# advait/c4a0

Hardware: AMD Instinct MI355X
Metric: self-play games/sec (and MCTS sims/sec) at n_mcts=100 (higher is better)
Workload: dtype bf16

## Files before the change

c4a0_amd/csrc/c4_head_gemm.hip:

```cpp
#include <hip/hip_runtime.h>
#include <stdint.h>

#include <string>
#include <type_traits>

#include "../../include/c4a0_hip.h"
#include "c4_grouped.hpp"
#include "c4_host.hpp"
#include "c4_timeline.hpp"

namespace {

typedef __bf16 bf16x8 __attribute__((ext_vector_type(8)));
typedef __bf16 bf16x4 __attribute__((ext_vector_type(4)));
typedef float f32x4 __attribute__((ext_vector_type(4)));

constexpr int BK = 64;

struct GemmParams {
  const uint16_t* x;
  const uint16_t* w;
  const float* bias;
  uint16_t* y;
  uint32_t M, N, K, ldx, ldy, relu;
  uint32_t xcd_mask, xcd_shift, xn_log2, rm, rn, rn_magic;
};

#define C4_GEMM_ARGS const uint16_t* __restrict__ a_x, const uint16_t* __restrict__ a_w, const float* __restrict__ a_bias, uint16_t* __restrict__ a_y, \
                     uint32_t a_m, uint32_t a_nk, uint32_t a_ld, uint32_t a_flags, uint32_t a_rmrn, uint32_t a_magic
#define C4_GEMM_UNPACK()                                                                                                              \
  GemmParams p;                                                                                                                        \
  p.x = a_x; p.w = a_w; p.bias = a_bias; p.y = a_y; p.M = a_m; p.N = a_nk & 0xFFFFu; p.K = a_nk >> 16; p.ldx = a_ld & 0xFFFFu;         \
  p.ldy = a_ld >> 16; p.relu = a_flags & 0xFFu; p.xn_log2 = (a_flags >> 8) & 0xFFu; p.xcd_mask = (a_flags >> 16) & 0xFFu;              \
  p.xcd_shift = a_flags >> 24; p.rm = a_rmrn & 0xFFFFu; p.rn = a_rmrn >> 16; p.rn_magic = a_magic

__host__ __device__ __forceinline__ void tile_of_block(uint32_t blk, uint32_t xcd_mask, uint32_t xcd_shift, uint32_t xn_log2, uint32_t rm, uint32_t rn,
                                                       uint32_t rn_magic, int& tm, int& tn) {
  const uint32_t xcd = blk & xcd_mask, idx = blk >> xcd_shift;
  const uint32_t qn = rn == 1u ? idx : (uint32_t)(((uint64_t)idx * rn_magic) >> 32);
  tm = (int)((xcd >> xn_log2) * rm + qn);
  tn = (int)((xcd & ((1u << xn_log2) - 1u)) * rn + (idx - qn * rn));
}

template <int N>
__device__ __forceinline__ void wait_vmcnt() { asm volatile("s_waitcnt vmcnt(%0)" ::"n"(N) : "memory"); }

#if defined(C4_PHASE_STAMPS) && !defined(C4_GEMM_CLOCK)
#define C4_GEMM_CLOCK
#endif
#ifdef C4_GEMM_CLOCK
__device__ unsigned long long c4_gemm_clk[16];
#define C4_CLK_DECL() unsigned long long clk_ts[8]; unsigned long long clk_c0 = 0, clk_c1 = 0
#define C4_GSTAMP(i) do { clk_ts[i] = __builtin_amdgcn_s_memrealtime(); } while (0)
#define C4_CLK_BEGIN() do { clk_c0 = __builtin_amdgcn_s_memtime(); } while (0)
#define C4_CLK_END() do { clk_c1 = __builtin_amdgcn_s_memtime(); } while (0)
#ifdef C4_PHASE_STAMPS
#define C4_CLK_SAMPLE() true
#else
#define C4_CLK_SAMPLE() ((blockIdx.x & 31) == 5)
#endif
#define C4_CLK_FLUSH()                                                                                       \
  do {                                                                                                       \
    if (threadIdx.x == 0 && C4_CLK_SAMPLE()) {                                                               \
      atomicAdd(&c4_gemm_clk[0], clk_c1 - clk_c0);                                                           \
      atomicAdd(&c4_gemm_clk[1], clk_ts[3] - clk_ts[1]);                                                     \
      atomicAdd(&c4_gemm_clk[2], 1ull);                                                                      \
      if (C4_CLK_PHASES) {                                                                                   \
        for (int i_ = 0; i_ < 7; i_++) atomicAdd(&c4_gemm_clk[4 + i_], clk_ts[i_ + 1] - clk_ts[i_]);         \
        atomicMin(&c4_gemm_clk[12], clk_ts[0]);                                                              \
        atomicMax(&c4_gemm_clk[13], clk_ts[7]);                                                              \
      }                                                                                                      \
    }                                                                                                        \
  } while (0)
#ifdef C4_PHASE_STAMPS
#define C4_CLK_PHASES 1
#else
#define C4_CLK_PHASES 0
#endif
#else
#define C4_CLK_DECL() do { } while (0)
#define C4_GSTAMP(i) do { } while (0)
#define C4_CLK_BEGIN() do { } while (0)
#define C4_CLK_END() do { } while (0)
#define C4_CLK_FLUSH() do { } while (0)
#endif


typedef uint32_t u32x4 __attribute__((ext_vector_type(4)));

__device__ __forceinline__ float relu1(float v) {
  float r;
  asm("v_max_f32 %0, 0, %1" : "=v"(r) : "v"(v));
  return r;
}

template <int TM, int TN, bool RELU>
__device__ __forceinline__ void store_wave_tile_impl(const f32x4 (&acc)[TN][TM], const f32x4 (&bias_v)[TN], const GemmParams& p, int m_wave0, int n_wave0,
                                                     int li, int lg) {
  auto finish = [&](const f32x4& a, const f32x4& bv) __attribute__((always_inline)) {
    f32x4 v = a + bv;
    if (RELU) {
#pragma unroll
      for (int r = 0; r < 4; r++) v[r] = relu1(v[r]);
    }
    return __builtin_bit_cast(uint2, __builtin_convertvector(v, bf16x4));
  };
  const int m16 = m_wave0 + 16 * (lg & 1) + li;
  uint16_t* y16 = p.y + (size_t)m16 * p.ldy + (n_wave0 + 8 * (lg >> 1));
  const size_t pair_step = (size_t)32 * p.ldy;
#pragma unroll
  for (int pb = 0; pb < TM / 2; pb++) {
#pragma unroll
    for (int a = 0; a < TN; a++) {
      const uint2 o0 = finish(acc[a][2 * pb], bias_v[a]), o1 = finish(acc[a][2 * pb + 1], bias_v[a]);
      const auto sx = __builtin_amdgcn_permlane16_swap(o0.x, o1.x, false, false);
      const auto sy = __builtin_amdgcn_permlane16_swap(o0.y, o1.y, false, false);
      const u32x4 v = {sx[0], sy[0], sx[1], sy[1]};
      if (m16 + 32 * pb < (int)p.M) *reinterpret_cast<u32x4*>(y16 + a * 16) = v;
    }
    y16 += pair_step;
  }
  if (TM & 1) {
    const int m8 = m_wave0 + 16 * (TM - 1) + li;
    uint16_t* y8 = p.y + (size_t)m8 * p.ldy + (n_wave0 + 4 * lg);
    if (m8 < (int)p.M) {
#pragma unroll
      for (int a = 0; a < TN; a++) *reinterpret_cast<uint2*>(y8 + a * 16) = finish(acc[a][TM - 1], bias_v[a]);
    }
  }
}

template <int TM, int TN>
__device__ __forceinline__ void store_wave_tile(const f32x4 (&acc)[TN][TM], const f32x4 (&bias_v)[TN], const GemmParams& p, int m_wave0, int n_wave0,
                                                int li, int lg) {
  if (p.relu) store_wave_tile_impl<TM, TN, true>(acc, bias_v, p, m_wave0, n_wave0, li, lg);
  else store_wave_tile_impl<TM, TN, false>(acc, bias_v, p, m_wave0, n_wave0, li, lg);
}

template <int BM, int BN, int WM, int WN, int NSTAGE, int MINW, int NLOAD = 0, int STAG = 0, int WST = 0, typename... GA>
__global__ __launch_bounds__(64 * (WM * WN + NLOAD), MINW) void c4_head_gemm_kernel(C4_GEMM_ARGS, GA... a_group) {
  C4_GEMM_UNPACK();
  constexpr int kWaves = WM * WN;
  constexpr int kIssuers = NLOAD ? NLOAD : kWaves;
  constexpr int TM = BM / WM / 16, TN = BN / WN / 16;
  constexpr int kStageBytes = (BM + BN) * BK * 2;
  constexpr int kChunks = (BM + BN) / 8;
  constexpr int L = kChunks / kIssuers;
  static_assert(kChunks % kIssuers == 0, "every issuing wavefront issues the same number of loads per k-tile (counted waits)");
  static_assert(BM % (16 * WM) == 0 && BN % (16 * WN) == 0, "wave tiles are multiples of 16");
  static_assert(NSTAGE >= 2 && NSTAGE <= 4, "ring depth");
  constexpr bool kSplit = WST != 0;
  constexpr int kXStage = BM * BK * 2, kWStage = BN * BK * 2;
  constexpr int LX = (BM / 8) / kIssuers, LW = L - LX;
  static_assert(!kSplit || (NLOAD == 0 && STAG == 0 && NSTAGE == 3 && WST == 2 && (BM / 8) % kIssuers == 0 && (BN / 8) % kIssuers == 0),
                "the split ring is written for three X stages + two W stages, every wavefront issuing whole shares of both");
  extern __shared__ __attribute__((aligned(1024))) uint8_t lds[];
  C4_CLK_DECL();
  C4_GSTAMP(0);
  C4_TL_BEGIN();

  const int tid = threadIdx.x, lane = tid & 63;
  const int wave = __builtin_amdgcn_readfirstlane(tid >> 6);
  const int wm = wave % WM, wn = (wave / WM) % WN;
  const int li = lane & 15, lg = lane >> 4;
  const bool is_loader = NLOAD != 0 && wave >= kWaves;
  const int issuer = NLOAD ? wave - kWaves : wave;

  int tm, tn;
  tile_of_block(blockIdx.x, p.xcd_mask, p.xcd_shift, p.xn_log2, p.rm, p.rn, p.rn_magic, tm, tn);
  const int tm0 = tm * BM, tn0 = tn * BN;
  if constexpr (sizeof...(GA) != 0) {
    const int model = c4grp::Segments{a_group...}.model_of((uint32_t)tm0);
    if (model < 0) return;
    p.w += (size_t)model * p.N * p.K;
    p.bias += (size_t)model * p.N;
  }

  uint32_t src_off[L];
  const int r8 = lane >> 3, slot = lane & 7;
#pragma unroll
  for (int i = 0; i < L; i++) {
    const int c = (issuer < 0 ? 0 : issuer) + kIssuers * i;
    if (c < BM / 8) {
      const int row = c * 8 + r8;
      int gr = tm0 + row;
      gr = gr < (int)p.M ? gr : (int)p.M - 1;
      src_off[i] = (uint32_t)gr * p.ldx * 2u + (uint32_t)((slot ^ (row & 7)) * 16);
    } else {
      const int row = (c - BM / 8) * 8 + r8;
      src_off[i] = (uint32_t)(tn0 + row) * p.K * 2u + (uint32_t)((slot ^ (row & 7)) * 16);
    }
  }
  const auto x_rsrc = __builtin_amdgcn_make_buffer_rsrc((void*)p.x, 0, (int)(((p.M - 1) * p.ldx + p.K) * 2u), 0x00020000);
  const auto w_rsrc = __builtin_amdgcn_make_buffer_rsrc((void*)p.w, 0, (int)(p.N * p.K * 2u), 0x00020000);
  const int KT = (int)p.K / BK;
  auto issue_one = [&](int kt, int i) __attribute__((always_inline)) {
    const int c = (issuer < 0 ? 0 : issuer) + kIssuers * i;
    uint8_t* dst = lds + (kt % NSTAGE) * kStageBytes + c * 1024;
    if (kSplit) dst = c < BM / 8 ? lds + (kt % NSTAGE) * kXStage + c * 1024 : lds + NSTAGE * kXStage + (kt % (kSplit ? WST : 1)) * kWStage + (c - BM / 8) * 1024;
    const uint32_t tail = kt >= KT ? 0x80000000u : 0u;
    __builtin_amdgcn_raw_ptr_buffer_load_lds((c < BM / 8) ? x_rsrc : w_rsrc, (__attribute__((address_space(3))) void*)dst, 16,
                                             (int)(src_off[i] | tail), kt * (BK * 2), 0, 0);
  };
  auto issue = [&](int kt) __attribute__((always_inline)) {
#pragma unroll
    for (int i = 0; i < L; i++) issue_one(kt, i);
  };
  if (NLOAD != 0 && is_loader) {
#pragma unroll
    for (int s = 0; s < NSTAGE - 1; s++) issue(s);
    for (int kt = 0; kt < KT; kt++) {
      wait_vmcnt<(NSTAGE - 2) * L>();
      __builtin_amdgcn_s_barrier();
      issue(kt + NSTAGE - 1);
    }
    wait_vmcnt<0>();
    return;
  }

  f32x4 acc[TN][TM];
#pragma unroll
  for (int a = 0; a < TN; a++)
#pragma unroll
    for (int b = 0; b < TM; b++) acc[a][b] = f32x4{0.f, 0.f, 0.f, 0.f};

  const uint32_t frag_off0 = (uint32_t)li * 128u + (uint32_t)(((0 + lg) ^ (li & 7)) * 16);
  const uint32_t frag_off1 = (uint32_t)li * 128u + (uint32_t)(((4 + lg) ^ (li & 7)) * 16);
  const uint32_t x_base = (uint32_t)(wm * (BM / WM)) * 128u;
  const uint32_t w_base = (uint32_t)(wn * (BN / WN)) * 128u;

  f32x4 bias_v[TN];
#pragma unroll
  for (int a = 0; a < TN; a++) bias_v[a] = *reinterpret_cast<const f32x4*>(p.bias + tn0 + wn * (BN / WN) + a * 16 + 4 * lg);
  if (NLOAD == 0 && !kSplit) {
#pragma unroll
    for (int s = 0; s < NSTAGE - 1; s++) issue(s);
  }
  if (kSplit) {
#pragma unroll
    for (int i = 0; i < LX; i++) issue_one(0, i);
#pragma unroll
    for (int i = LX; i < L; i++) issue_one(0, i);
#pragma unroll
    for (int i = 0; i < LX; i++) issue_one(1, i);
  }

  C4_GSTAMP(1);
  C4_CLK_BEGIN();
  static_assert(!STAG || (NLOAD == 0 && WM * WN == 8 && NSTAGE >= 3), "the stagger is written for 8 computing wavefronts that issue their own pieces");
  bf16x8 afr[2][TN], bfr[2][TM];
  auto body = [&](int kt, auto late_c) __attribute__((always_inline)) {
    constexpr bool kLate = decltype(late_c)::value;
    if (kSplit) wait_vmcnt<LX>();
    else if (NLOAD == 0) wait_vmcnt<(NSTAGE - 2) * L>();
    __builtin_amdgcn_s_barrier();
#ifdef C4_GEMM_CLOCK
    if (kt == 0) C4_GSTAMP(2);
#endif
    const int lkt = kt + NSTAGE - 1;
    constexpr int kLoadSteps = NSTAGE == 2 ? TN : 2 * TN;
    constexpr int kLoadsPerStep = (L + kLoadSteps - 1) / kLoadSteps;
    const uint8_t* stx = kSplit ? lds + (kt % NSTAGE) * kXStage : lds + (kt % NSTAGE) * kStageBytes;
    const uint8_t* stw = kSplit ? lds + NSTAGE * kXStage + (kt % (kSplit ? WST : 1)) * kWStage : stx + kXStage;
    auto rd_x = [&](int kk, int b) __attribute__((always_inline)) {
      bfr[kk][b] = *reinterpret_cast<const bf16x8*>(stx + x_base + (kk ? frag_off1 : frag_off0) + b * 2048);
    };
    auto rd_w = [&](int kk, int a) __attribute__((always_inline)) {
      afr[kk][a] = *reinterpret_cast<const bf16x8*>(stw + w_base + (kk ? frag_off1 : frag_off0) + a * 2048);
    };
    auto issue_step = [&](int step) __attribute__((always_inline)) {
      if (NLOAD == 0 && (NSTAGE >= 3 || step < TN)) {
#pragma unroll
        for (int j = step * kLoadsPerStep; j < (step + 1) * kLoadsPerStep && j < L; j++) {
          if (!kSplit) issue_one(lkt, j);
          else if (j < LW) issue_one(kt + WST - 1, LX + j);
          else issue_one(kt + NSTAGE - 1, j - LW);
        }
      }
    };
#pragma unroll
    for (int b = 0; b < TM; b++) rd_x(0, b);
#pragma unroll
    for (int a = 0; a < TN; a++) rd_w(0, a);
    __builtin_amdgcn_sched_barrier(0);
    constexpr int kPerStep = (TN + TM + TN - 1) / TN;
    if (kLate) {
#pragma unroll
      for (int a = 0; a < TN; a++) {
        if (kt > 0) {
#pragma unroll
          for (int b = 0; b < TM; b++) acc[a][b] = __builtin_amdgcn_mfma_f32_16x16x32_bf16(afr[1][a], bfr[1][b], acc[a][b], 0, 0, 0);
        }
        issue_step(a);
        __builtin_amdgcn_sched_barrier(0);
      }
    }
#pragma unroll
    for (int a = 0; a < TN; a++) {
#pragma unroll
      for (int b = 0; b < TM; b++) acc[a][b] = __builtin_amdgcn_mfma_f32_16x16x32_bf16(afr[0][a], bfr[0][b], acc[a][b], 0, 0, 0);
#pragma unroll
      for (int r = a * kPerStep; r < (a + 1) * kPerStep && r < TN + TM; r++) {
        if (r < TM) rd_x(1, r); else rd_w(1, r - TM);
      }
      issue_step(kLate ? TN + a : a);
      __builtin_amdgcn_sched_barrier(0);
    }
    if (kLate) {
      asm volatile("s_waitcnt lgkmcnt(0)" ::: "memory");
    } else {
#pragma unroll
      for (int a = 0; a < TN; a++) {
#pragma unroll
        for (int b = 0; b < TM; b++) acc[a][b] = __builtin_amdgcn_mfma_f32_16x16x32_bf16(afr[1][a], bfr[1][b], acc[a][b], 0, 0, 0);
        issue_step(TN + a);
        __builtin_amdgcn_sched_barrier(0);
      }
    }
  };
  if (STAG && wave >= kWaves / 2) {
    for (int kt = 0; kt < KT; kt++) body(kt, std::true_type{});
#pragma unroll
    for (int a = 0; a < TN; a++)
#pragma unroll
      for (int b = 0; b < TM; b++) acc[a][b] = __builtin_amdgcn_mfma_f32_16x16x32_bf16(afr[1][a], bfr[1][b], acc[a][b], 0, 0, 0);
  } else {
    for (int kt = 0; kt < KT; kt++) body(kt, std::false_type{});
  }

  C4_CLK_END();
  C4_GSTAMP(3);
  wait_vmcnt<0>();
  C4_GSTAMP(4);
#pragma unroll
  for (int a = 0; a < TN; a++) asm volatile("" ::"v"(bias_v[a]));
  C4_GSTAMP(5);
  store_wave_tile<TM, TN>(acc, bias_v, p, tm0 + wm * (BM / WM), tn0 + wn * (BN / WN), li, lg);
  C4_GSTAMP(6);
#ifdef C4_GEMM_CLOCK
  if (C4_CLK_PHASES) wait_vmcnt<0>();
  C4_GSTAMP(7);
  C4_CLK_FLUSH();
#endif
  C4_TL_END(2, p.y);
}

template <int BM, int BN, int WM, int WN, int NSTAGE, int MINW = 1>
__global__ __launch_bounds__(64 * WM * WN, MINW) void c4_head_gemm32_kernel(C4_GEMM_ARGS) {
  C4_GEMM_UNPACK();
  constexpr int BKT = 32;
  constexpr int kWaves = WM * WN;
  constexpr int TM = BM / WM / 16, TN = BN / WN / 16;
  constexpr int kStageBytes = (BM + BN) * BKT * 2;
  constexpr int kChunks = (BM + BN) / 16;
  constexpr int L = (kChunks + kWaves - 1) / kWaves;
  constexpr int R = kChunks % kWaves;
  static_assert(BM % (16 * WM) == 0 && BN % (16 * WN) == 0 && NSTAGE >= 3 && NSTAGE <= 5, "tile / ring");
  extern __shared__ __attribute__((aligned(1024))) uint8_t lds[];

  const int tid = threadIdx.x, lane = tid & 63;
  const int wave = __builtin_amdgcn_readfirstlane(tid >> 6);
  const int wm = wave % WM, wn = wave / WM;
  const int li = lane & 15, lg = lane >> 4;
  const bool short_wave = R != 0 && wave >= R;

  int tm, tn;
  tile_of_block(blockIdx.x, p.xcd_mask, p.xcd_shift, p.xn_log2, p.rm, p.rn, p.rn_magic, tm, tn);
  const int tm0 = tm * BM, tn0 = tn * BN;

  auto swz = [](int row) __attribute__((always_inline)) { return (0x78 >> (2 * ((row >> 2) & 3))) & 3; };
  uint32_t src_off[L];
  const int r16 = lane >> 2, slot = lane & 3;
#pragma unroll
  for (int i = 0; i < L; i++) {
    int c = wave + kWaves * i;
    c = c < kChunks ? c : kChunks - 1;
    if (c < BM / 16) {
      const int row = c * 16 + r16;
      int gr = tm0 + row;
      gr = gr < (int)p.M ? gr : (int)p.M - 1;
      src_off[i] = (uint32_t)gr * p.ldx * 2u + (uint32_t)((slot ^ swz(row)) * 16);
    } else {
      const int row = (c - BM / 16) * 16 + r16;
      src_off[i] = (uint32_t)(tn0 + row) * p.K * 2u + (uint32_t)((slot ^ swz(row)) * 16);
    }
  }
  const auto x_rsrc = __builtin_amdgcn_make_buffer_rsrc((void*)p.x, 0, (int)(((p.M - 1) * p.ldx + p.K) * 2u), 0x00020000);
  const auto w_rsrc = __builtin_amdgcn_make_buffer_rsrc((void*)p.w, 0, (int)(p.N * p.K * 2u), 0x00020000);
  const int KT = (int)p.K / BKT;
  auto issue_one = [&](int kt, int i) __attribute__((always_inline)) {
    if (i == L - 1 && short_wave) return;
    uint8_t* st = lds + (kt % NSTAGE) * kStageBytes;
    const int c = wave + kWaves * i;
    const uint32_t tail = kt >= KT ? 0x80000000u : 0u;
    __builtin_amdgcn_raw_ptr_buffer_load_lds((c < BM / 16) ? x_rsrc : w_rsrc, (__attribute__((address_space(3))) void*)(st + c * 1024), 16,
                                             (int)(src_off[i] | tail), kt * (BKT * 2), 0, 0);
  };
  auto wait_tile = [&]() __attribute__((always_inline)) {
    if (short_wave) wait_vmcnt<(NSTAGE - 2) * (L - 1)>(); else wait_vmcnt<(NSTAGE - 2) * L>();
    asm volatile("s_waitcnt lgkmcnt(0)" ::: "memory");
  };

  f32x4 acc[TN][TM];
#pragma unroll
  for (int a = 0; a < TN; a++)
#pragma unroll
    for (int b = 0; b < TM; b++) acc[a][b] = f32x4{0.f, 0.f, 0.f, 0.f};

  const uint32_t frag_off = (uint32_t)li * 64u + (uint32_t)((lg ^ swz(li)) * 16);
  const uint32_t x_base = (uint32_t)(wm * (BM / WM)) * 64u;
  const uint32_t w_base = (uint32_t)(BM * BKT * 2) + (uint32_t)(wn * (BN / WN)) * 64u;

  f32x4 bias_v[TN];
#pragma unroll
  for (int a = 0; a < TN; a++) bias_v[a] = *reinterpret_cast<const f32x4*>(p.bias + tn0 + wn * (BN / WN) + a * 16 + 4 * lg);
#pragma unroll
  for (int s = 0; s < NSTAGE - 1; s++) {
#pragma unroll
    for (int i = 0; i < L; i++) issue_one(s, i);
  }

  bf16x8 afr[2][TN], bfr[2][TM];
  auto read_frags = [&](int kt, int f) __attribute__((always_inline)) {
    const uint8_t* st = lds + (kt % NSTAGE) * kStageBytes;
#pragma unroll
    for (int b = 0; b < TM; b++) bfr[f][b] = *reinterpret_cast<const bf16x8*>(st + x_base + frag_off + b * 1024);
#pragma unroll
    for (int a = 0; a < TN; a++) afr[f][a] = *reinterpret_cast<const bf16x8*>(st + w_base + frag_off + a * 1024);
  };
  constexpr int kLoadsPerStep = (L + TN - 1) / TN;
  auto step = [&](int kt, int fcur, int fprev, bool do_mfma) __attribute__((always_inline)) {
    wait_tile();
    __builtin_amdgcn_s_barrier();
    read_frags(kt, fcur);
    __builtin_amdgcn_sched_barrier(0);
#pragma unroll
    for (int a = 0; a < TN; a++) {
      if (do_mfma) {
#pragma unroll
        for (int b = 0; b < TM; b++) acc[a][b] = __builtin_amdgcn_mfma_f32_16x16x32_bf16(afr[fprev][a], bfr[fprev][b], acc[a][b], 0, 0, 0);
      }
#pragma unroll
      for (int j = a * kLoadsPerStep; j < (a + 1) * kLoadsPerStep && j < L; j++) issue_one(kt + NSTAGE - 1, j);
      __builtin_amdgcn_sched_barrier(0);
    }
  };
  step(0, 0, 1, false);
  for (int kt = 1; kt + 1 < KT; kt += 2) {
    step(kt, 1, 0, true);
    step(kt + 1, 0, 1, true);
  }
  step(KT - 1, 1, 0, true);
#pragma unroll
  for (int a = 0; a < TN; a++)
#pragma unroll
    for (int b = 0; b < TM; b++) acc[a][b] = __builtin_amdgcn_mfma_f32_16x16x32_bf16(afr[1][a], bfr[1][b], acc[a][b], 0, 0, 0);
  wait_vmcnt<0>();

#pragma unroll
  for (int a = 0; a < TN; a++) asm volatile("" ::"v"(bias_v[a]));
  store_wave_tile<TM, TN>(acc, bias_v, p, tm0 + wm * (BM / WM), tn0 + wn * (BN / WN), li, lg);
}

template <int BM, int BN>
__global__ __launch_bounds__(256, 1) void c4_head_gemm4_kernel(C4_GEMM_ARGS) {
  C4_GEMM_UNPACK();
  constexpr int WM = 2, WN = 2;
  constexpr int TM = BM / WM / 16, TN = BN / WN / 16;
  constexpr int kStageBytes = (BM + BN) * BK * 2;
  constexpr int kChunks = (BM + BN) / 8;
  constexpr int L = kChunks / 4;
  static_assert(kChunks % 4 == 0 && (BM / 8) % 4 == 0, "every wavefront moves whole shares of both operands");
  constexpr int LX = (BM / 8) / 4;
  extern __shared__ __attribute__((aligned(1024))) uint8_t lds[];

  const int tid = threadIdx.x, lane = tid & 63;
  const int wave = __builtin_amdgcn_readfirstlane(tid >> 6);
  const int wm = wave % WM, wn = wave / WM;
  const int li = lane & 15, lg = lane >> 4;
  int tm, tn;
  tile_of_block(blockIdx.x, p.xcd_mask, p.xcd_shift, p.xn_log2, p.rm, p.rn, p.rn_magic, tm, tn);
  const int tm0 = tm * BM, tn0 = tn * BN;

  uint32_t src_off[L], dst_off[L];
  const int r8 = lane >> 3, slot = lane & 7;
#pragma unroll
  for (int i = 0; i < L; i++) {
    const bool is_x = i < LX;
    const int c = is_x ? wave + 4 * i : wave + 4 * (i - LX);
    const int row = c * 8 + r8;
    if (is_x) {
      int gr = tm0 + row;
      gr = gr < (int)p.M ? gr : (int)p.M - 1;
      src_off[i] = (uint32_t)gr * p.ldx * 2u + (uint32_t)(slot * 16);
      dst_off[i] = (uint32_t)row * 128u + (uint32_t)((slot ^ (row & 7)) * 16);
    } else {
      src_off[i] = (uint32_t)(tn0 + row) * p.K * 2u + (uint32_t)(slot * 16);
      dst_off[i] = (uint32_t)(BM + row) * 128u + (uint32_t)((slot ^ (row & 7)) * 16);
    }
  }
  const auto x_rsrc = __builtin_amdgcn_make_buffer_rsrc((void*)p.x, 0, (int)(((p.M - 1) * p.ldx + p.K) * 2u), 0x00020000);
  const auto w_rsrc = __builtin_amdgcn_make_buffer_rsrc((void*)p.w, 0, (int)(p.N * p.K * 2u), 0x00020000);
  const int KT = (int)p.K / BK;
  u32x4 stg[L];
  auto load_tile = [&](int kt) __attribute__((always_inline)) {
    const uint32_t tail = kt >= KT ? 0x80000000u : 0u;
#pragma unroll
    for (int i = 0; i < L; i++)
      stg[i] = __builtin_amdgcn_raw_buffer_load_b128(i < LX ? x_rsrc : w_rsrc, (int)(src_off[i] | tail), kt * (BK * 2), 0);
  };
  auto store_tile = [&](int kt) __attribute__((always_inline)) {
    uint8_t* st = lds + (kt & 1) * kStageBytes;
#pragma unroll
    for (int i = 0; i < L; i++) *reinterpret_cast<u32x4*>(st + dst_off[i]) = stg[i];
  };

  f32x4 acc[TN][TM];
#pragma unroll
  for (int a = 0; a < TN; a++)
#pragma unroll
    for (int b = 0; b < TM; b++) acc[a][b] = f32x4{0.f, 0.f, 0.f, 0.f};
  const uint32_t frag_off0 = (uint32_t)li * 128u + (uint32_t)(((0 + lg) ^ (li & 7)) * 16);
  const uint32_t frag_off1 = (uint32_t)li * 128u + (uint32_t)(((4 + lg) ^ (li & 7)) * 16);
  const uint32_t x_base = (uint32_t)(wm * (BM / WM)) * 128u;
  const uint32_t w_base = (uint32_t)(BM + wn * (BN / WN)) * 128u;
  f32x4 bias_v[TN];
#pragma unroll
  for (int a = 0; a < TN; a++) bias_v[a] = *reinterpret_cast<const f32x4*>(p.bias + tn0 + wn * (BN / WN) + a * 16 + 4 * lg);

  load_tile(0);
  store_tile(0);
  load_tile(1);
  bf16x8 afr[2][TN], bfr[2][TM];
  for (int kt = 0; kt < KT; kt++) {
    asm volatile("s_waitcnt lgkmcnt(0)" ::: "memory");
    __builtin_amdgcn_s_barrier();
    const uint8_t* st = lds + (kt & 1) * kStageBytes;
    auto rd_x = [&](int kk, int b) __attribute__((always_inline)) {
      bfr[kk][b] = *reinterpret_cast<const bf16x8*>(st + x_base + (kk ? frag_off1 : frag_off0) + b * 2048);
    };
    auto rd_w = [&](int kk, int a) __attribute__((always_inline)) {
      afr[kk][a] = *reinterpret_cast<const bf16x8*>(st + w_base + (kk ? frag_off1 : frag_off0) + a * 2048);
    };
#pragma unroll
    for (int b = 0; b < TM; b++) rd_x(0, b);
#pragma unroll
    for (int a = 0; a < TN; a++) rd_w(0, a);
    __builtin_amdgcn_sched_barrier(0);
    store_tile(kt + 1);
    load_tile(kt + 2);
    __builtin_amdgcn_sched_barrier(0);
    constexpr int kPerStep = (TN + TM + TN - 1) / TN;
#pragma unroll
    for (int a = 0; a < TN; a++) {
#pragma unroll
      for (int b = 0; b < TM; b++) acc[a][b] = __builtin_amdgcn_mfma_f32_16x16x32_bf16(afr[0][a], bfr[0][b], acc[a][b], 0, 0, 0);
#pragma unroll
      for (int r = a * kPerStep; r < (a + 1) * kPerStep && r < TN + TM; r++) {
        if (r < TM) rd_x(1, r); else rd_w(1, r - TM);
      }
      __builtin_amdgcn_sched_barrier(0);
    }
#pragma unroll
    for (int a = 0; a < TN; a++) {
#pragma unroll
      for (int b = 0; b < TM; b++) acc[a][b] = __builtin_amdgcn_mfma_f32_16x16x32_bf16(afr[1][a], bfr[1][b], acc[a][b], 0, 0, 0);
      __builtin_amdgcn_sched_barrier(0);
    }
  }
#pragma unroll
  for (int a = 0; a < TN; a++) asm volatile("" ::"v"(bias_v[a]));
  store_wave_tile<TM, TN>(acc, bias_v, p, tm0 + wm * (BM / WM), tn0 + wn * (BN / WN), li, lg);
}

inline uint32_t set_tile_order(GemmParams& p, uint32_t tiles_m, uint32_t tiles_n, uint32_t bm, uint32_t bn) {
  p.xcd_mask = 0; p.xcd_shift = 0; p.xn_log2 = 0; p.rm = tiles_m; p.rn = tiles_n;
  uint64_t best = ~0ull;
  for (uint32_t xm = 1, l2 = 3; xm <= 8; xm *= 2, l2--) {
    const uint32_t xn = 8 / xm;
    if (tiles_m % xm || tiles_n % xn) continue;
    const uint64_t rows = (uint64_t)(tiles_m / xm) * bm + (uint64_t)(tiles_n / xn) * bn;
    if (rows < best) { best = rows; p.xcd_mask = 7; p.xcd_shift = 3; p.xn_log2 = l2; p.rm = tiles_m / xm; p.rn = tiles_n / xn; }
  }
  p.rn_magic = p.rn == 1 ? 0u : (uint32_t)((1ull << 32) / p.rn + 1);
  return tiles_m * tiles_n;
}

template <int BM, int BN, typename K, typename... GA>
int launch_common(K k, GemmParams p, int threads, int lds_bytes, hipStream_t stream, int device, GA... group) {
  if (lds_bytes > 64 * 1024) {
    const hipError_t e = c4host::opt_in_lds((const void*)k, lds_bytes, device);
    if (e != hipSuccess) return c4host::fail(C4_ERR_HIP, std::string("c4_linear_bf16: LDS opt-in: ") + hipGetErrorString(e));
  }
  const uint32_t tiles = set_tile_order(p, (p.M + BM - 1) / BM, p.N / BN, BM, BN);
  if (p.rm > 0xFFFFu || p.rn > 0xFFFFu)
    return c4host::fail(C4_ERR_BAD_ARG, "c4_linear_bf16: more than 65 535 tiles along one dimension of an XCD's rectangle (m too large for this tile)");
  k<<<dim3(tiles), dim3(threads), lds_bytes, stream>>>(p.x, p.w, p.bias, p.y, p.M, p.N | (p.K << 16), p.ldx | (p.ldy << 16),
                                                         (p.relu ? 1u : 0u) | (p.xn_log2 << 8) | (p.xcd_mask << 16) | (p.xcd_shift << 24), p.rm | (p.rn << 16), p.rn_magic, group...);
  const hipError_t e = hipGetLastError();
  if (e != hipSuccess) return c4host::fail(C4_ERR_HIP, std::string("c4_linear_bf16 launch: ") + hipGetErrorString(e));
  return C4_OK;
}

template <int BM, int BN, int WM, int WN, int NSTAGE, int MINW = 1>
int launch_gemm32(GemmParams p, hipStream_t stream, int device) {
  return launch_common<BM, BN>(c4_head_gemm32_kernel<BM, BN, WM, WN, NSTAGE, MINW>, p, 64 * WM * WN, NSTAGE * (BM + BN) * 32 * 2, stream, device);
}

template <int BM, int BN, int WM, int WN, int NSTAGE, int MINW, int NLOAD = 0, int STAG = 0, int WST = 0>
int launch_gemm(GemmParams p, hipStream_t stream, int device) {
  return launch_common<BM, BN>(c4_head_gemm_kernel<BM, BN, WM, WN, NSTAGE, MINW, NLOAD, STAG, WST>, p, 64 * (WM * WN + NLOAD),
                               WST ? (NSTAGE * BM + WST * BN) * BK * 2 : NSTAGE * (BM + BN) * BK * 2, stream, device);
}

}

#ifdef C4_GEMM_CLOCK
extern "C" int c4_debug_gemm_clock(double* ghz, double* loop_us, uint64_t* n_workgroups, int reset) {
  unsigned long long h[16];
  if (hipDeviceSynchronize() != hipSuccess || hipMemcpyFromSymbol(h, HIP_SYMBOL(c4_gemm_clk), sizeof h) != hipSuccess) return C4_ERR_HIP;
  if (ghz) *ghz = h[1] ? (double)h[0] / (double)h[1] * 0.1 : 0.0;
  if (loop_us) *loop_us = h[2] ? (double)h[1] / (double)h[2] * 0.01 : 0.0;
  if (n_workgroups) *n_workgroups = h[2];
  if (reset) { unsigned long long z[16] = {0}; z[12] = ~0ull; if (hipMemcpyToSymbol(HIP_SYMBOL(c4_gemm_clk), z, sizeof z) != hipSuccess) return C4_ERR_HIP; }
  return C4_OK;
}
extern "C" int c4_debug_gemm_phases(double* phase_us, double* span_us, int reset) {
  unsigned long long h[16];
  if (hipDeviceSynchronize() != hipSuccess || hipMemcpyFromSymbol(h, HIP_SYMBOL(c4_gemm_clk), sizeof h) != hipSuccess) return C4_ERR_HIP;
  for (int i = 0; i < 7; i++) phase_us[i] = h[2] ? (double)h[4 + i] / (double)h[2] * 0.01 : 0.0;
  if (span_us) *span_us = h[13] > h[12] ? (double)(h[13] - h[12]) * 0.01 : 0.0;
  if (reset) { unsigned long long z[16] = {0}; z[12] = ~0ull; if (hipMemcpyToSymbol(HIP_SYMBOL(c4_gemm_clk), z, sizeof z) != hipSuccess) return C4_ERR_HIP; }
  return C4_OK;
}
#endif

C4_TL_SETTER(c4_debug_timeline_gemm)

extern "C" int c4_linear_bf16_tile_map(uint32_t m, uint32_t n, uint32_t bm, uint32_t bn, uint32_t* tiles_out, uint32_t cap_blocks, uint32_t* n_blocks) {
  if (!n_blocks || bm == 0 || bn == 0 || m == 0 || n == 0 || n % bn) return c4host::fail(C4_ERR_BAD_ARG, "c4_linear_bf16_tile_map: bad argument");
  GemmParams p{};
  p.M = m; p.N = n;
  const uint32_t tiles = set_tile_order(p, (m + bm - 1) / bm, n / bn, bm, bn);
  *n_blocks = tiles;
  if (p.rm > 0xFFFFu || p.rn > 0xFFFFu) return c4host::fail(C4_ERR_BAD_ARG, "c4_linear_bf16_tile_map: more than 65 535 tiles along one dimension");
  if (!tiles_out) return C4_OK;
  if (cap_blocks < tiles) return c4host::fail(C4_ERR_BAD_ARG, "c4_linear_bf16_tile_map: output too small");
  for (uint32_t b = 0; b < tiles; b++) {
    int tm, tn;
    tile_of_block(b, p.xcd_mask, p.xcd_shift, p.xn_log2, p.rm, p.rn, p.rn_magic, tm, tn);
    tiles_out[2 * b] = (uint32_t)tm; tiles_out[2 * b + 1] = (uint32_t)tn;
  }
  return C4_OK;
}

extern "C" int c4_linear_bf16(const void* x_dev, const void* w_dev, const float* bias_dev, void* y_dev, uint32_t m, uint32_t n,
                              uint32_t k, uint32_t ldx, uint32_t ldy, uint32_t relu, uint32_t config, void* stream) {
  if (!x_dev || !w_dev || !bias_dev || !y_dev) return c4host::fail(C4_ERR_BAD_ARG, "c4_linear_bf16: null argument");
  if (k == 0 || k % BK) return c4host::fail(C4_ERR_BAD_ARG, "c4_linear_bf16: K must be a positive multiple of 64");
  if (n == 0 || n % 192) return c4host::fail(C4_ERR_BAD_ARG, "c4_linear_bf16: N must be a positive multiple of 192 (42 x C features, C a multiple of 32)");
  if (ldx < k || ldy < n || ldx % 8 || ldy % 8 || ((uintptr_t)y_dev & 15) || ((uintptr_t)x_dev & 15))
    return c4host::fail(C4_ERR_BAD_ARG, "c4_linear_bf16: row strides must cover a row and keep rows 16-byte aligned (x and y)");
  if ((uint64_t)m * ldx * 2 >= (1ull << 31) || (uint64_t)n * k * 2 >= (1ull << 31)) return c4host::fail(C4_ERR_BAD_ARG, "c4_linear_bf16: operands are addressed with 31-bit byte offsets (< 2 GiB each)");
  if (n >= 65536 || k >= 65536 || ldx >= 65536 || ldy >= 65536) return c4host::fail(C4_ERR_BAD_ARG, "c4_linear_bf16: n, k and the row strides must be below 65 536 (packed kernel arguments)");
  if (m == 0) return C4_OK;
  const int device = c4host::stream_device((hipStream_t)stream);
  c4host::DeviceGuard guard(device);
  if (guard.error() != hipSuccess) return c4host::fail(C4_ERR_HIP, std::string("c4_linear_bf16: hipSetDevice: ") + hipGetErrorString(guard.error()));
  GemmParams p{(const uint16_t*)x_dev, (const uint16_t*)w_dev, bias_dev, (uint16_t*)y_dev, m, n, k, ldx, ldy, relu, 0, 0, 0, 0, 0, 0};
  hipStream_t st = (hipStream_t)stream;
  if (config == 0) {
    const bool wide = n > k;
    config = m <= 384 ? 27 : m <= 640 ? (wide ? 9 : 27) : m <= 896 ? (wide ? 23 : 9) : m <= 1024 ? (wide ? 10 : 9) : 11;
    if (k >= 2048) config = m <= 384 ? (wide ? 9 : 27) : m <= 640 ? (wide ? 10 : 9) : m <= 1024 ? (wide ? 11 : 10) : 7;
  }
  switch (config) {
    case 1: return launch_gemm<128, 192, 2, 2, 2, 2>(p, st, device);
    case 2: return launch_gemm<128, 192, 2, 4, 4, 1>(p, st, device);
    case 3: return launch_gemm<256, 192, 2, 4, 2, 1>(p, st, device);
    case 4: return launch_gemm<128, 96, 2, 2, 2, 2>(p, st, device);
    case 5: return launch_gemm<64, 192, 1, 4, 2, 2>(p, st, device);
    case 6: return launch_gemm<128, 192, 2, 2, 3, 1>(p, st, device);
    case 7: return launch_gemm<256, 192, 4, 2, 2, 1>(p, st, device);
    case 8: return launch_gemm<128, 96, 2, 2, 4, 1>(p, st, device);
    case 9: return launch_gemm<64, 96, 2, 2, 4, 2>(p, st, device);
    case 10: return launch_gemm<128, 96, 2, 2, 3, 1>(p, st, device);
    case 11: return launch_gemm<128, 192, 2, 4, 3, 1>(p, st, device);
    case 12: return launch_gemm<128, 192, 1, 4, 3, 1>(p, st, device);
    case 13: return launch_gemm<128, 192, 2, 2, 4, 1>(p, st, device);
    case 14: return launch_gemm<256, 96, 2, 2, 3, 1>(p, st, device);
    case 15: return launch_gemm<64, 192, 1, 4, 3, 1>(p, st, device);
    case 16: return launch_gemm<64, 192, 2, 4, 3, 1>(p, st, device);
    case 17: return launch_gemm32<256, 192, 2, 4, 4>(p, st, device);
    case 18: return launch_gemm32<256, 192, 2, 4, 3>(p, st, device);
    case 19: return launch_gemm32<256, 192, 4, 2, 4>(p, st, device);
    case 20: return launch_gemm<128, 192, 2, 4, 2, 2>(p, st, device);
    case 21: return launch_gemm<96, 192, 2, 2, 3, 1>(p, st, device);
    case 22: return launch_gemm<96, 96, 2, 2, 4, 1>(p, st, device);
    case 23: return launch_gemm<96, 96, 2, 2, 3, 1>(p, st, device);
    case 24: return launch_gemm<96, 192, 2, 2, 4, 1>(p, st, device);
    case 25: return launch_gemm<96, 96, 2, 3, 3, 1>(p, st, device);
    case 26: return launch_gemm<192, 96, 2, 2, 2, 1>(p, st, device);
    case 27: return launch_gemm<64, 64, 2, 2, 4, 2>(p, st, device);
    case 28: return launch_gemm<96, 64, 2, 2, 3, 1>(p, st, device);
    case 29: return launch_gemm<192, 192, 2, 4, 3, 1>(p, st, device);
    case 30: return launch_gemm<192, 192, 4, 2, 3, 1>(p, st, device);
    case 31: return launch_gemm32<256, 192, 4, 2, 5>(p, st, device);
    case 32: return launch_gemm32<256, 192, 2, 4, 5>(p, st, device);
    case 33: return launch_gemm<192, 96, 2, 2, 4, 1>(p, st, device);
    case 34: return launch_gemm<192, 192, 2, 2, 3, 1>(p, st, device);
    case 35: return launch_gemm<128, 192, 2, 4, 3, 1, 4>(p, st, device);
    case 36: return launch_gemm<128, 192, 2, 4, 4, 1, 4>(p, st, device);
    case 37: return launch_gemm<128, 192, 2, 2, 3, 1, 4>(p, st, device);
    case 38: return launch_gemm<128, 192, 2, 4, 3, 1, 2>(p, st, device);
    case 39: return launch_gemm<128, 192, 2, 4, 3, 1, 8>(p, st, device);
    case 40: return launch_gemm<96, 96, 2, 2, 3, 1, 2>(p, st, device);
    case 41: return launch_gemm<64, 64, 2, 2, 4, 2, 2>(p, st, device);
    case 42: return launch_gemm<64, 96, 2, 2, 4, 2, 2>(p, st, device);
    case 43: return launch_gemm<128, 96, 2, 2, 3, 1, 2>(p, st, device);
    case 44: return launch_gemm<96, 96, 2, 2, 3, 1, 4>(p, st, device);
    case 45: return launch_gemm<64, 64, 2, 2, 4, 2, 4>(p, st, device);
    case 46: return launch_gemm<128, 192, 2, 4, 3, 1, 0, 1>(p, st, device);
    case 47: return launch_gemm<128, 192, 2, 4, 4, 1, 0, 1>(p, st, device);
    case 48: return launch_gemm<256, 192, 4, 2, 3, 1, 0, 0, 2>(p, st, device);
    case 49: return launch_gemm<256, 192, 2, 2, 3, 1, 0, 0, 2>(p, st, device);
    case 50: return launch_gemm32<128, 192, 2, 4, 4, 4>(p, st, device);
    case 51: return launch_gemm32<128, 192, 2, 4, 3, 4>(p, st, device);
    case 52: return launch_gemm32<128, 192, 2, 2, 4, 2>(p, st, device);
    case 54: return launch_gemm<96, 192, 2, 2, 3, 1, 4>(p, st, device);
    case 55: return launch_gemm<96, 192, 2, 4, 3, 1, 4>(p, st, device);
    case 56: return launch_gemm<192, 96, 2, 2, 3, 1, 4>(p, st, device);
    case 57: return launch_gemm<192, 96, 4, 2, 3, 1, 4>(p, st, device);
    case 58: return launch_gemm<192, 96, 2, 2, 4, 1, 4>(p, st, device);
    case 59: return launch_gemm<192, 96, 2, 2, 3, 1, 2>(p, st, device);
    case 53: return launch_common<256, 192>(c4_head_gemm4_kernel<256, 192>, p, 256, 2 * (256 + 192) * BK * 2, st, device);
    default: return c4host::fail(C4_ERR_BAD_ARG, "c4_linear_bf16: unknown config");
  }
}

extern "C" int c4_linear_bf16_grouped(const void* x_dev, const void* w_dev, const float* bias_dev, void* y_dev, const uint32_t* seg_start_dev, uint32_t n_models,
                                      uint32_t rows_cap, uint32_t n, uint32_t k, uint32_t ldx, uint32_t ldy, uint32_t relu, void* stream) {
  if (!x_dev || !w_dev || !bias_dev || !y_dev || !seg_start_dev) return c4host::fail(C4_ERR_BAD_ARG, "c4_linear_bf16_grouped: null argument");
  if (k == 0 || k % BK) return c4host::fail(C4_ERR_BAD_ARG, "c4_linear_bf16_grouped: K must be a positive multiple of 64");
  if (n == 0 || n % 192) return c4host::fail(C4_ERR_BAD_ARG, "c4_linear_bf16_grouped: N must be a positive multiple of 192 (42 x C features, C a multiple of 32)");
  if (ldx < k || ldy < n || ldx % 8 || ldy % 8 || ((uintptr_t)y_dev & 15) || ((uintptr_t)x_dev & 15))
    return c4host::fail(C4_ERR_BAD_ARG, "c4_linear_bf16_grouped: row strides must cover a row and keep rows 16-byte aligned (x and y)");
  if ((uint64_t)rows_cap * ldx * 2 >= (1ull << 31) || (uint64_t)n * k * 2 >= (1ull << 31))
    return c4host::fail(C4_ERR_BAD_ARG, "c4_linear_bf16_grouped: operands are addressed with 31-bit byte offsets (< 2 GiB; the weights: each model's layer)");
  if (n >= 65536 || k >= 65536 || ldx >= 65536 || ldy >= 65536) return c4host::fail(C4_ERR_BAD_ARG, "c4_linear_bf16_grouped: n, k and the row strides must be below 65 536 (packed kernel arguments)");
  if (n_models == 0 || n_models > C4_ROUTE_MAX_MODELS) return c4host::fail(C4_ERR_BAD_ARG, "c4_linear_bf16_grouped: n_models must be between 1 and C4_ROUTE_MAX_MODELS");
  if (rows_cap % C4_GROUPED_ROW_ALIGN) return c4host::fail(C4_ERR_BAD_ARG, "c4_linear_bf16_grouped: rows_cap must be a multiple of C4_GROUPED_ROW_ALIGN");
  if (rows_cap == 0) return C4_OK;
  const int device = c4host::stream_device((hipStream_t)stream);
  c4host::DeviceGuard guard(device);
  if (guard.error() != hipSuccess) return c4host::fail(C4_ERR_HIP, std::string("c4_linear_bf16_grouped: hipSetDevice: ") + hipGetErrorString(guard.error()));
  GemmParams p{(const uint16_t*)x_dev, (const uint16_t*)w_dev, bias_dev, (uint16_t*)y_dev, rows_cap, n, k, ldx, ldy, relu, 0, 0, 0, 0, 0, 0};
  static_assert(C4_GROUPED_ROW_ALIGN % 128 == 0, "no GEMM workgroup straddles two segments");
  return launch_common<128, 192>(c4_head_gemm_kernel<128, 192, 2, 4, 3, 1, 0, 0, 0, const uint32_t*, uint32_t>, p, 64 * 8, 3 * (128 + 192) * BK * 2, (hipStream_t)stream,
                                 device, seg_start_dev, n_models);
}
```

Measured before the change: 28730.

## Add uneven load-share GEMM variant with 16 waves and route large wide heads to it

```diff
diff --git a/c4a0_amd/csrc/c4_head_gemm.hip b/c4a0_amd/csrc/c4_head_gemm.hip
--- a/c4a0_amd/csrc/c4_head_gemm.hip
+++ b/c4a0_amd/csrc/c4_head_gemm.hip
@@ -145,14 +145,17 @@
   constexpr int TM = BM / WM / 16, TN = BN / WN / 16;
   constexpr int kStageBytes = (BM + BN) * BK * 2;
   constexpr int kChunks = (BM + BN) / 8;
-  constexpr int L = kChunks / kIssuers;
-  static_assert(kChunks % kIssuers == 0, "every issuing wavefront issues the same number of loads per k-tile (counted waits)");
+  constexpr bool kUneven = kChunks % kIssuers != 0;
+  constexpr int kHeavy = kUneven ? kIssuers / 2 : kIssuers;
+  constexpr int L = kUneven ? (BM / 8) / kIssuers + (BN / 8) / kHeavy : kChunks / kIssuers;
+  static_assert(!kUneven || (NLOAD == 0 && sizeof...(GA) == 0 && (BM / 8) % kIssuers == 0 && (BN / 8) % kHeavy == 0 && kHeavy % 4 == 0),
+                "uneven shares: whole shares of X for every wavefront, whole shares of W for half of them, the same number on every SIMD");
   static_assert(BM % (16 * WM) == 0 && BN % (16 * WN) == 0, "wave tiles are multiples of 16");
   static_assert(NSTAGE >= 2 && NSTAGE <= 4, "ring depth");
   constexpr bool kSplit = WST != 0;
   constexpr int kXStage = BM * BK * 2, kWStage = BN * BK * 2;
-  constexpr int LX = (BM / 8) / kIssuers, LW = L - LX;
-  static_assert(!kSplit || (NLOAD == 0 && STAG == 0 && NSTAGE == 3 && WST == 2 && (BM / 8) % kIssuers == 0 && (BN / 8) % kIssuers == 0),
+  constexpr int LX = (BM / 8) / kIssuers;
+  static_assert(!kSplit || (NLOAD == 0 && (STAG == 0 || kUneven) && NSTAGE == 3 && WST == 2 && (BM / 8) % kIssuers == 0 && (kUneven || (BN / 8) % kIssuers == 0)),
                 "the split ring is written for three X stages + two W stages, every wavefront issuing whole shares of both");
   extern __shared__ __attribute__((aligned(1024))) uint8_t lds[];
   C4_CLK_DECL();
@@ -165,6 +168,11 @@
   const int li = lane & 15, lg = lane >> 4;
   const bool is_loader = NLOAD != 0 && wave >= kWaves;
   const int issuer = NLOAD ? wave - kWaves : wave;
+  const bool has_w = !kUneven || issuer < kHeavy;
+  auto piece_of = [&](int i) __attribute__((always_inline)) {
+    const int w = issuer < 0 ? 0 : issuer;
+    return kUneven && i >= LX ? BM / 8 + (w & (kHeavy - 1)) + kHeavy * (i - LX) : w + kIssuers * i;
+  };
 
   int tm, tn;
   tile_of_block(blockIdx.x, p.xcd_mask, p.xcd_shift, p.xn_log2, p.rm, p.rn, p.rn_magic, tm, tn);
@@ -180,7 +188,7 @@
   const int r8 = lane >> 3, slot = lane & 7;
 #pragma unroll
   for (int i = 0; i < L; i++) {
-    const int c = (issuer < 0 ? 0 : issuer) + kIssuers * i;
+    const int c = piece_of(i);
     if (c < BM / 8) {
       const int row = c * 8 + r8;
       int gr = tm0 + row;
@@ -195,16 +203,20 @@
   const auto w_rsrc = __builtin_amdgcn_make_buffer_rsrc((void*)p.w, 0, (int)(p.N * p.K * 2u), 0x00020000);
   const int KT = (int)p.K / BK;
   auto issue_one = [&](int kt, int i) __attribute__((always_inline)) {
-    const int c = (issuer < 0 ? 0 : issuer) + kIssuers * i;
+    const int c = piece_of(i);
     uint8_t* dst = lds + (kt % NSTAGE) * kStageBytes + c * 1024;
     if (kSplit) dst = c < BM / 8 ? lds + (kt % NSTAGE) * kXStage + c * 1024 : lds + NSTAGE * kXStage + (kt % (kSplit ? WST : 1)) * kWStage + (c - BM / 8) * 1024;
     const uint32_t tail = kt >= KT ? 0x80000000u : 0u;
-    __builtin_amdgcn_raw_ptr_buffer_load_lds((c < BM / 8) ? x_rsrc : w_rsrc, (__attribute__((address_space(3))) void*)dst, 16,
+    __builtin_amdgcn_raw_ptr_buffer_load_lds((kUneven ? i < LX : c < BM / 8) ? x_rsrc : w_rsrc, (__attribute__((address_space(3))) void*)dst, 16,
                                              (int)(src_off[i] | tail), kt * (BK * 2), 0, 0);
   };
   auto issue = [&](int kt) __attribute__((always_inline)) {
 #pragma unroll
-    for (int i = 0; i < L; i++) issue_one(kt, i);
+    for (int i = 0; i < LX; i++) issue_one(kt, i);
+    if (has_w) {
+#pragma unroll
+      for (int i = LX; i < L; i++) issue_one(kt, i);
+    }
   };
   if (NLOAD != 0 && is_loader) {
 #pragma unroll
@@ -239,27 +251,30 @@
   if (kSplit) {
 #pragma unroll
     for (int i = 0; i < LX; i++) issue_one(0, i);
-#pragma unroll
-    for (int i = LX; i < L; i++) issue_one(0, i);
+    if (has_w) {
+#pragma unroll
+      for (int i = LX; i < L; i++) issue_one(0, i);
+    }
 #pragma unroll
     for (int i = 0; i < LX; i++) issue_one(1, i);
   }
 
   C4_GSTAMP(1);
   C4_CLK_BEGIN();
-  static_assert(!STAG || (NLOAD == 0 && WM * WN == 8 && NSTAGE >= 3), "the stagger is written for 8 computing wavefronts that issue their own pieces");
+  static_assert(!STAG || (NLOAD == 0 && ((WM * WN == 8 && NSTAGE >= 3) || kUneven)), "the stagger is written for 8 computing wavefronts that issue their own pieces, and for the 16 of the uneven form (whose late half are the light wavefronts)");
   bf16x8 afr[2][TN], bfr[2][TM];
-  auto body = [&](int kt, auto late_c) __attribute__((always_inline)) {
+  auto body = [&](int kt, auto late_c, auto light_c) __attribute__((always_inline)) {
     constexpr bool kLate = decltype(late_c)::value;
+    constexpr int Lk = decltype(light_c)::value ? LX : L, LWk = Lk - LX;
     if (kSplit) wait_vmcnt<LX>();
-    else if (NLOAD == 0) wait_vmcnt<(NSTAGE - 2) * L>();
+    else if (NLOAD == 0) wait_vmcnt<(NSTAGE - 2) * Lk>();
     __builtin_amdgcn_s_barrier();
 #ifdef C4_GEMM_CLOCK
     if (kt == 0) C4_GSTAMP(2);
 #endif
     const int lkt = kt + NSTAGE - 1;
     constexpr int kLoadSteps = NSTAGE == 2 ? TN : 2 * TN;
-    constexpr int kLoadsPerStep = (L + kLoadSteps - 1) / kLoadSteps;
+    constexpr int kLoadsPerStep = (Lk + kLoadSteps - 1) / kLoadSteps;
     const uint8_t* stx = kSplit ? lds + (kt % NSTAGE) * kXStage : lds + (kt % NSTAGE) * kStageBytes;
     const uint8_t* stw = kSplit ? lds + NSTAGE * kXStage + (kt % (kSplit ? WST : 1)) * kWStage : stx + kXStage;
     auto rd_x = [&](int kk, int b) __attribute__((always_inline)) {
@@ -271,10 +286,10 @@
     auto issue_step = [&](int step) __attribute__((always_inline)) {
       if (NLOAD == 0 && (NSTAGE >= 3 || step < TN)) {
 #pragma unroll
-        for (int j = step * kLoadsPerStep; j < (step + 1) * kLoadsPerStep && j < L; j++) {
+        for (int j = step * kLoadsPerStep; j < (step + 1) * kLoadsPerStep && j < Lk; j++) {
           if (!kSplit) issue_one(lkt, j);
-          else if (j < LW) issue_one(kt + WST - 1, LX + j);
-          else issue_one(kt + NSTAGE - 1, j - LW);
+          else if (j < LWk) issue_one(kt + WST - 1, LX + j);
+          else issue_one(kt + NSTAGE - 1, j - LWk);
         }
       }
     };
@@ -319,13 +334,15 @@
     }
   };
   if (STAG && wave >= kWaves / 2) {
-    for (int kt = 0; kt < KT; kt++) body(kt, std::true_type{});
+    for (int kt = 0; kt < KT; kt++) body(kt, std::true_type{}, std::integral_constant<bool, kUneven>{});
 #pragma unroll
     for (int a = 0; a < TN; a++)
 #pragma unroll
       for (int b = 0; b < TM; b++) acc[a][b] = __builtin_amdgcn_mfma_f32_16x16x32_bf16(afr[1][a], bfr[1][b], acc[a][b], 0, 0, 0);
+  } else if (kUneven && !has_w) {
+    for (int kt = 0; kt < KT; kt++) body(kt, std::false_type{}, std::true_type{});
   } else {
-    for (int kt = 0; kt < KT; kt++) body(kt, std::false_type{});
+    for (int kt = 0; kt < KT; kt++) body(kt, std::false_type{}, std::false_type{});
   }
 
   C4_CLK_END();
@@ -672,6 +689,7 @@
   if (config == 0) {
     const bool wide = n > k;
     config = m <= 384 ? 27 : m <= 640 ? (wide ? 9 : 27) : m <= 896 ? (wide ? 23 : 9) : m <= 1024 ? (wide ? 10 : 9) : 11;
+    if (wide && m >= 2304) config = 61;
     if (k >= 2048) config = m <= 384 ? (wide ? 9 : 27) : m <= 640 ? (wide ? 10 : 9) : m <= 1024 ? (wide ? 11 : 10) : 7;
   }
   switch (config) {
@@ -733,6 +751,10 @@
     case 57: return launch_gemm<192, 96, 4, 2, 3, 1, 4>(p, st, device);
     case 58: return launch_gemm<192, 96, 2, 2, 4, 1, 4>(p, st, device);
     case 59: return launch_gemm<192, 96, 2, 2, 3, 1, 2>(p, st, device);
+    case 60: return launch_gemm<256, 192, 4, 4, 3, 1, 0, 0, 2>(p, st, device);
+    case 61: return launch_gemm<256, 192, 4, 4, 2, 1>(p, st, device);
+    case 62: return launch_gemm<256, 192, 4, 4, 3, 1, 0, 1, 2>(p, st, device);
+    case 63: return launch_gemm<256, 192, 4, 4, 2, 1, 0, 1>(p, st, device);
     case 53: return launch_common<256, 192>(c4_head_gemm4_kernel<256, 192>, p, 256, 2 * (256 + 192) * BK * 2, st, device);
     default: return c4host::fail(C4_ERR_BAD_ARG, "c4_linear_bf16: unknown config");
   }
```

After: 28740 (median of 5 runs). About the same (+0.0%).
